# CasualGANPapers/Make-A-Scene

Hardware: AMD Instinct MI355X
Metric: VQ-IMG 256x256 images/sec/node (recon+VQ fwd+bwd) (higher is better)
Workload: dtype bf16; 1 GPU; VQ-IMG 256x256, codebook 8192x256, conf/img_config.yaml model block (95.2 M params), fwd+bwd of L1+q_loss + Adam step; per_gpu_batch=32, global_batch=32, parallelism=dp1, optimizer=mas_hip.optim.Adam (one launch; = torch.optim.Adam's update)

## Files before the change

### include/mas_hip.h

```cpp
#ifndef MAS_HIP_H
#define MAS_HIP_H

#include <stddef.h>
#include <stdint.h>

#ifdef __cplusplus
extern "C" {
#endif

#define MAS_ABI_VERSION 10

enum { MAS_OK = 0, MAS_EINVAL = -1, MAS_EUNSUPPORTED = -2, MAS_ELAUNCH = -3, MAS_EWORKSPACE = -4 };
enum { MAS_F32 = 0, MAS_BF16 = 1 };
enum { MAS_ACT_NONE = 0,
       MAS_ACT_AFFINE = 1,
       MAS_ACT_AFFINE_SILU = 2  };

typedef struct MasConvDesc {
    int32_t N, H, W, Cin;
    int32_t Ho, Wo, Cout;
    int32_t ks;
    int32_t stride;
    int32_t pad_top, pad_left;
    int32_t in_dtype;
    int32_t out_dtype;
    int32_t act;
    int32_t upsample;
    int32_t w_layout;
    int32_t wgrad_cus;
} MasConvDesc;

int         mas_abi_version(void);
const char* mas_last_error(void);
const char* mas_last_kernel(void);

size_t mas_packed_weight_elems(int Cout, int Cin, int ks);
int    mas_pack_conv_weight(const float* w_oihw, void* packed, int Cout, int Cin, int ks,
                            int transpose, int dtype, void* stream);
enum { MAS_WLAYOUT_K64 = 0, MAS_WLAYOUT_K32 = 1, MAS_WLAYOUT_UP2 = 2 };
size_t mas_packed_weight_elems_up2(int Cout, int Cin);
int    mas_conv_weight_layout(const MasConvDesc* d);
int    mas_pack_conv_weight_layout(const float* w_oihw, void* packed, int Cout, int Cin, int ks,
                                   int transpose, int dtype, int layout, void* stream);

typedef struct MasPackItem {
    const float* w_oihw; void* packed;
    int Cout, Cin, ks, transpose, dtype, layout, first_block, n_blocks;
} MasPackItem;
int    mas_pack_batch_blocks(int Cout, int Cin, int ks, int transpose, int dtype, int layout);
int    mas_pack_conv_weight_batch(const MasPackItem* items_device, int n_items, int total_blocks, void* stream);

typedef struct MasPackTileItem {
    const float* w_oihw; void* img[4];
    int transpose[4], layout[4];
    int n_img, Cout, Cin, ks, first_block, pad_;
} MasPackTileItem;
int    mas_pack_tile_blocks(int Cout, int Cin, int ks);
int    mas_pack_conv_weight_tiles(const MasPackTileItem* items_device, int n_items, int total_blocks, int max_ks, void* stream);

typedef struct MasAdamItem {
    float* p; const float* g; float* m; float* v;
    long long n;
    int first_block, pad_;
} MasAdamItem;
int    mas_adam_blocks(long long numel);
int    mas_adam_multi(const MasAdamItem* items_device, int n_items, int total_blocks, float lr, float beta1, float beta2, float eps,
                      float weight_decay, double bias_correction1, double bias_correction2, void* stream);

int    mas_grad_sqnorm_multi(const MasAdamItem* items_device, int n_items, int total_blocks, double* partials, void* stream);
int    mas_grad_clip_coef(const double* partials, int n_partials, const double* extra, int n_extra, float max_norm, float* out, void* stream);
int    mas_adam_multi_ex(const MasAdamItem* items_device, int n_items, int total_blocks, float lr, float beta1, float beta2, float eps,
                         float weight_decay, double bias_correction1, double bias_correction2, const float* grad_scale_device,
                         int decoupled_wd, void* stream);
int    mas_grad_scale_multi(const MasAdamItem* items_device, int n_items, int total_blocks, const float* scale_device, void* stream);

int    mas_adam_multi_ema(const MasAdamItem* items_device, float* const* ema_device, int n_items, int total_blocks, float lr, float beta1,
                          float beta2, float eps, float weight_decay, double bias_correction1, double bias_correction2,
                          const float* grad_scale_device, int decoupled_wd, float ema_decay, const float* grad_norm_device, void* stream);
int    mas_swap_multi(const MasAdamItem* items_device, float* const* other_device, int n_items, int total_blocks, void* stream);

int    mas_adam_multi_dev(const MasAdamItem* items_device, float* const* ema_device, const float* const* step_device, int n_items,
                          int total_blocks, const float* lr_device, double beta1, double beta2, float eps, float weight_decay,
                          const float* grad_scale_device, int decoupled_wd, double ema_decay, const float* ema_count_device,
                          const float* grad_norm_device, float* scalars_device, void* stream);
int    mas_adam_advance_dev(float* counters, int n, void* stream);

size_t mas_gn_stats_workspace(int N, int C);
int    mas_gn_stats(const void* x, int dtype, int N, int HW, int C, int G, float eps,
// ... 267 lines not shown
int mas_obj_head_grid_dev(int level, int max_cells, int n_canvas, int H, int W);
int mas_obj_canvas_fwd_dev(const MasFaceImage* img, const MasFaceImage* rec, const int32_t* table_dev, int max_cells, int n_images,
                           int n_canvas, int H, int W, const float* shift, const float* scale, void* canvas, int dtype, void* stream);
int mas_obj_canvas_bwd_dev(const void* dcanvas, int dtype, const int32_t* table_dev, int max_cells, int n_images, int n_canvas, int H, int W,
                           const float* scale, const MasFaceImage* drec, void* stream);
int mas_obj_relu_fwd_dev(void* y, const int32_t* table_dev, int max_cells, int n_images, int n_canvas, int H, int W, int level, int N, int C,
                         int dtype, void* stream);
int mas_obj_pool_fwd_dev(const void* x, void* y, const int32_t* table_dev, int max_cells, int n_images, int n_canvas, int H, int W, int level,
                         int N, int C, int dtype, void* stream);
int mas_obj_pool_bwd_dev(const void* a, const void* seed, const void* dz, void* dy, const int32_t* table_dev, int max_cells, int n_images,
                         int n_canvas, int H, int W, int level, int N, int C, int dtype, void* stream);
int mas_obj_head_fwd_dev(const void* feat, const float* w, const int32_t* table_dev, int max_cells, int n_images, int n_canvas, int H, int W,
                         int level, int dtype, float* partial, void* stream);
int mas_obj_finalize_dev(const float* partial, const int32_t* table_dev, int max_cells, int n_images, int n_canvas, int H, int W, float* out,
                         void* stream);
int mas_obj_head_bwd_dev(const void* feat, const float* w, const int32_t* table_dev, int max_cells, int n_images, int n_canvas, int H, int W,
                         int level, int dtype, const float* dout, void* seed, void* stream);

int mas_lpips_pack_fwd(const MasFaceImage* real, const MasFaceImage* fake, const float* shift, const float* scale, void* canvas, int dtype,
                       void* stream);
int mas_lpips_pack_bwd(const void* dcanvas, int dtype, const float* scale, const MasFaceImage* dfake, void* stream);
int mas_lpips_relu_fwd(void* y, long long n, int dtype, void* stream);
int mas_lpips_pool_fwd(const void* x, void* y, int N, int H, int W, int C, int dtype, void* stream);
int mas_lpips_pool_bwd(const void* a, const void* seed, const void* dz, void* dy, int N, int H, int W, int C, int dtype, void* stream);
int mas_lpips_head_blocks(int H, int W, int C);
int mas_lpips_head_fwd(const void* feat, const float* w, int B, int H, int W, int C, int dtype, float* partial, void* stream);
int mas_lpips_finalize(const float* partial, int B, int n_levels, const int32_t* hw, const int32_t* blocks, float* out, void* stream);
int mas_lpips_head_bwd(const void* feat, const float* w, int B, int H, int W, int C, int dtype, const float* dout, void* seed, void* stream);

#define MAS_RESERVOIR_PER_IMAGE 10
#define MAS_RESERVOIR_MAX_CANDIDATES 2048
int mas_reservoir_collect(const float* z, float* buf, int32_t* state, int32_t* plan, long long seed, int R, int B, int HW, int D,
                          void* stream);

size_t mas_kmeans_workspace(int M, int K);
int mas_kmeans_init(const float* points, int M, int K, int D, long long seed, int draw, float* centroids, int32_t* init_idx, void* stream);
int mas_kmeans_fit(const float* points, float* centroids, int M, int K, int D, int max_iter, float tol, int64_t* assign, int32_t* info,
                   double* shift, void* workspace, size_t ws_bytes, void* stream);

enum { MAS_GAN_RUN = 8 };
int mas_gan_l1_blocks(int N, int C, int H, int W);
int mas_gan_l1_fwd(const void* img, int img_dtype, int img_layout, const void* rec, int rec_dtype, int rec_layout, int N, int C, int H,
                   int W, double* partials, int n_partials, void* stream);
int mas_gan_l1_finalize(const double* partials, int n_partials, long long numel, const float* perceptual, int B, float perceptual_weight,
                        float* out, void* stream);
int mas_gan_l1_bwd(const void* img, int img_dtype, int img_layout, const void* rec, int rec_dtype, int rec_layout, int N, int C, int H,
                   int W, const float* grad, void* drec, float* dperceptual, int B, float perceptual_weight, void* stream);
int mas_gan_logits_fwd(const float* fake, long long n_fake, const float* real, long long n_real, const long long* global_step,
                       long long disc_start, float disc_factor, float* out, void* stream);
int mas_gan_logits_bwd(const float* fake, long long n_fake, const float* real, long long n_real, const float* grad_gen, const float* grad_d,
                       const float* gate, float* dfake, float* dreal, void* stream);
int mas_gan_combine_fwd(const float* nll, const float* g_loss, const float* codebook, long long n_codebook, const float* face,
                        const float* object, const float* nll_grads, const float* g_grads, long long n_grads, long long* global_step,
                        long long disc_start, float disc_factor, float disc_weight, float codebook_weight, int advance, float* out,
                        void* stream);
int mas_gan_combine_bwd(const float* grad, const float* out, float codebook_weight, long long n_codebook, float* grads, void* stream);

#ifdef __cplusplus
}
#endif
#endif
```

### make-a-scene_amd/csrc/misc.hip

```cpp
#include "mas_common.h"
#include <stdarg.h>

static thread_local char g_err[512] = "";

void mas_set_error(const char* fmt, ...) {
    va_list ap;
    va_start(ap, fmt);
    vsnprintf(g_err, sizeof(g_err), fmt, ap);
    va_end(ap);
}

int mas_num_cus() {
    static std::atomic<int> cus[64];
    int dev = 0;
    if (hipGetDevice(&dev) != hipSuccess) return 256;
    int c = cus[dev & 63].load(std::memory_order_relaxed);
    if (c == 0) {
        int n = 0;
        c = (hipDeviceGetAttribute(&n, hipDeviceAttributeMultiprocessorCount, dev) == hipSuccess && n > 0) ? n : 256;
        cus[dev & 63].store(c, std::memory_order_relaxed);
    }
    return c;
}

// ... 122 lines not shown
    const int b = blockIdx.x;
    while (lo < hi) {
        const int mid = (lo + hi + 1) >> 1;
        if (items[mid].first_block <= b) lo = mid; else hi = mid - 1;
    }
    const MasPackItem it = items[lo];
    const long long first = (long long)(b - it.first_block) * NT + threadIdx.x, stride = (long long)it.n_blocks * NT;
    const int rows = it.transpose ? it.Cin : it.Cout, cols = it.transpose ? it.Cout : it.Cin;
    const int rows_pad = (rows + 127) / 128 * 128;
    auto cdiv = [](int a, int d) { return (a + d - 1) / d; };
    if (it.layout == MAS_WLAYOUT_UP2)
        pack_weight_up2_body(it.w_oihw, (bf16_t*)it.packed, it.Cout, it.Cin, it.transpose, rows_pad, cdiv(cols, 32), first, stride);
    else if (it.layout == MAS_WLAYOUT_K32)
        pack_weight_k32_body(it.w_oihw, (bf16_t*)it.packed, it.Cout, it.Cin, it.ks, it.transpose, rows_pad, cdiv(cols, 32), first, stride);
    else if (it.dtype == MAS_BF16)
        pack_weight_body<bf16_t>(it.w_oihw, (bf16_t*)it.packed, it.Cout, it.Cin, it.ks, it.transpose, rows_pad, cdiv(cols, 64), first, stride);
    else
        pack_weight_body<float>(it.w_oihw, (float*)it.packed, it.Cout, it.Cin, it.ks, it.transpose, rows_pad, cdiv(cols, 32), first, stride);
}

__device__ __forceinline__ unsigned pk2(const bf16_t* l, int a, int b) {
    return (unsigned)reinterpret_cast<const unsigned short*>(l)[a] | ((unsigned)reinterpret_cast<const unsigned short*>(l)[b] << 16);
}
__global__ __launch_bounds__(NT) void pack_weight_tiles_kernel(const MasPackTileItem* __restrict__ items, int n_items) {
    extern __shared__ __attribute__((aligned(16))) unsigned char tsm[];
    bf16_t* L = reinterpret_cast<bf16_t*>(tsm);
    int lo = 0, hi = n_items - 1;
    const int b = blockIdx.x, tid = threadIdx.x;
    while (lo < hi) {
        const int mid = (lo + hi + 1) >> 1;
        if (items[mid].first_block <= b) lo = mid; else hi = mid - 1;
    }
    const MasPackTileItem it = items[lo];
    const int Cout = it.Cout, Cin = it.Cin, kk = it.ks * it.ks;
    const int tiles_i = (Cin + 127) / 128 * 2;
    const int tb = b - it.first_block, o0 = (tb / tiles_i) * 64, i0 = (tb % tiles_i) * 64;
    const int run = 64 * kk;
    const bool full = i0 + 64 <= Cin && ((size_t)Cin * kk) % 4 == 0 && (reinterpret_cast<uintptr_t>(it.w_oihw) & 15) == 0;
    if (full) {
        const int v4 = run / 4;
        for (int u = tid; u < 64 * v4; u += NT) {
            const int ol = u / v4, q = u - ol * v4;
            f32x4 v = {0.0f, 0.0f, 0.0f, 0.0f};
            if (o0 + ol < Cout) v = *reinterpret_cast<const f32x4*>(it.w_oihw + ((size_t)(o0 + ol) * Cin + i0) * kk + 4 * q);
            const bf16x4 o = {(bf16_t)v[0], (bf16_t)v[1], (bf16_t)v[2], (bf16_t)v[3]};
            *reinterpret_cast<bf16x4*>(L + (size_t)ol * run + 4 * q) = o;
        }
    } else {
        const int valid = i0 < Cin ? (Cin - i0 < 64 ? Cin - i0 : 64) * kk : 0;
        for (int u = tid; u < 64 * run; u += NT) {
            const int ol = u / run, f = u - ol * run;
            float v = 0.0f;
            if (o0 + ol < Cout && f < valid) v = it.w_oihw[((size_t)(o0 + ol) * Cin + i0) * kk + f];
            L[u] = (bf16_t)v;
        }
    }
    __syncthreads();
    for (int im = 0; im < it.n_img; ++im) {
        const int tr = it.transpose[im], k32 = it.layout[im] == MAS_WLAYOUT_K32;
        const int rows = tr ? Cin : Cout, cols = tr ? Cout : Cin;
        const int r0 = tr ? i0 : o0, c0 = tr ? o0 : i0;
        const int rows_pad = (rows + 127) / 128 * 128;
        if (r0 >= rows_pad) continue;
        unsigned char* out = reinterpret_cast<unsigned char*>(it.img[im]);
        if (!k32) {
            const int ch = c0 / 64;
            if (ch >= (cols + 63) / 64) continue;
            for (int u = tid; u < kk * 512; u += NT) {
                const int t = u >> 9, row_l = (u >> 3) & 63, sp = u & 7;
                const int row = r0 + row_l, ls = sp ^ ((row >> 1) & 7);
                const int ts = tr ? kk - 1 - t : t;
                u32x4 o;
#pragma unroll
                for (int e = 0; e < 4; ++e) {
                    const int ca = ls * 8 + 2 * e, cb = ca + 1;
                    const int ia = tr ? (ca * 64 + row_l) * kk + ts : (row_l * 64 + ca) * kk + ts;
                    const int ib = tr ? (cb * 64 + row_l) * kk + ts : (row_l * 64 + cb) * kk + ts;
                    o[e] = pk2(L, ia, ib);
                }
                *reinterpret_cast<u32x4*>(out + ((size_t)(ch * kk + t) * rows_pad + row) * 128 + sp * 16) = o;
            }
        } else {
            const int half = (r0 >> 6) & 1, base = r0 & ~127;
            for (int h = 0; h < 2; ++h) {
                const int ch = c0 / 32 + h;
                if (ch >= (cols + 31) / 32) continue;
                for (int u = tid; u < kk * 256; u += NT) {
                    const int t = u >> 8, i_ = (u >> 6) & 3, l16 = (u >> 2) & 15, sp = u & 3;
                    const int row = base + 32 * i_ + l16 + 16 * half;
                    const int row_l = 4 * l16 + i_;
                    const int ls = sp ^ ((row >> 2) & 3);
                    const int ts = tr ? kk - 1 - t : t;
                    u32x4 o;
#pragma unroll
                    for (int e = 0; e < 4; ++e) {
                        const int ca = h * 32 + ls * 8 + 2 * e, cb = ca + 1;
                        const int ia = tr ? (ca * 64 + row_l) * kk + ts : (row_l * 64 + ca) * kk + ts;
                        const int ib = tr ? (cb * 64 + row_l) * kk + ts : (row_l * 64 + cb) * kk + ts;
                        o[e] = pk2(L, ia, ib);
                    }
                    *reinterpret_cast<u32x4*>(out + ((size_t)(ch * kk + t) * rows_pad + row) * 64 + sp * 16) = o;
                }
            }
        }
    }
}

template <typename T>
__global__ __launch_bounds__(NT) void upsample2x_kernel(const T* __restrict__ x, T* __restrict__ y, int N, int H, int W, int C) {
    constexpr int EPU = 16 / (int)sizeof(T);
    const int upp = C / EPU;
    const long long total = (long long)N * 2 * H * 2 * W * upp;
    for (long long i = (long long)blockIdx.x * NT + threadIdx.x; i < total; i += (long long)gridDim.x * NT) {
// ... 380 lines not shown
```

### make-a-scene_amd/csrc/reservoir.hip

```cpp
#include "mas_common.h"
#include "mas_philox.h"

#define RSV_THREADS 256

MAS_HD uint32_t rsv_half_bits(uint32_t N);
#include "mas_bijection.h"

__device__ __forceinline__ int rsv_scan(int mine, int* s_scan) {
    __syncthreads();
    s_scan[threadIdx.x] = mine;
    __syncthreads();
    if (threadIdx.x == 0) {
        int run = 0;
        for (int i = 0; i < RSV_THREADS; ++i) { const int v = s_scan[i]; s_scan[i] = run; run += v; }
    }
    __syncthreads();
    return s_scan[threadIdx.x];
}

__global__ __launch_bounds__(RSV_THREADS) void reservoir_plan_kernel(int* __restrict__ state, int* __restrict__ plan, uint32_t k0, uint32_t k1,
                                                                     int R, int B, int HW) {
    __shared__ int s_drop[MAS_RESERVOIR_MAX_CANDIDATES];
    __shared__ int s_old[MAS_RESERVOIR_MAX_CANDIDATES];
    __shared__ int s_list[MAS_RESERVOIR_MAX_CANDIDATES];
// ... 40 lines not shown
    const int i = blockIdx.x * (RSV_THREADS / 64) + (threadIdx.x >> 6), lane = threadIdx.x & 63;
    if (i >= n) return;
    const int dst = plan[2 * i], src = plan[2 * i + 1];
    if (dst < 0 || dst >= R || src < 0 || src >= rows) return;
    const f32x4* from = reinterpret_cast<const f32x4*>(z + (size_t)src * D);
    f32x4* to = reinterpret_cast<f32x4*>(buf + (size_t)dst * D);
    for (int q = lane; q < D / 4; q += 64) to[q] = from[q];
}

extern "C" int mas_reservoir_collect(const float* z, float* buf, int32_t* state, int32_t* plan, long long seed, int R, int B, int HW, int D,
                                     void* stream) {
    MAS_ENTER();
    if (HW < MAS_RESERVOIR_PER_IMAGE) MAS_FAIL(MAS_EINVAL, "reservoir_collect: %d latent positions, fewer than the %d drawn per image", HW,
                                               MAS_RESERVOIR_PER_IMAGE);
    if (B <= 0 || R <= 0 || (long long)MAS_RESERVOIR_PER_IMAGE * B > R)
        MAS_FAIL(MAS_EINVAL, "reservoir_collect: %d candidates per call (10 * B, B=%d) exceed the reservoir's %d rows", 10 * B, B, R);
    if (D <= 0 || D % 4) MAS_FAIL(MAS_EINVAL, "reservoir_collect: D=%d is not a positive multiple of 4 (16-byte row copies)", D);
    if (MAS_RESERVOIR_PER_IMAGE * B > MAS_RESERVOIR_MAX_CANDIDATES)
        MAS_FAIL(MAS_EUNSUPPORTED, "reservoir_collect: B=%d gives more than %d candidates per call", B, MAS_RESERVOIR_MAX_CANDIDATES);
    if ((long long)R + MAS_RESERVOIR_PER_IMAGE * B > (1ll << 30) || (long long)B * HW > (1ll << 30))
        MAS_FAIL(MAS_EUNSUPPORTED, "reservoir_collect: R=%d, B*HW=%lld beyond 2^30 rows", R, (long long)B * HW);
    if (!z || !buf || !state || !plan) MAS_FAIL(MAS_EINVAL, "reservoir_collect: null argument");
    if (((uintptr_t)z | (uintptr_t)buf) & 15) MAS_FAIL(MAS_EINVAL, "reservoir_collect: z and buf must be 16-byte aligned");
    const int n = MAS_RESERVOIR_PER_IMAGE * B;
    hipStream_t s = reinterpret_cast<hipStream_t>(stream);
    hipLaunchKernelGGL(reservoir_plan_kernel, dim3(1), dim3(RSV_THREADS), 0, s, state, plan, (uint32_t)((unsigned long long)seed & 0xffffffffu),
                       (uint32_t)((unsigned long long)seed >> 32), R, B, HW);
    MAS_CHECK_LAUNCH("reservoir_plan");
    hipLaunchKernelGGL(reservoir_copy_kernel, dim3(mas_cdiv(n, RSV_THREADS / 64)), dim3(RSV_THREADS), 0, s, z, buf, plan, n, R,
                       (long long)B * HW, D);
    MAS_CHECK_LAUNCH("reservoir_copy");
    return MAS_OK;
}
```

### make-a-scene_amd/mas_hip/__init__.py

```python
from __future__ import annotations

import ctypes as C
import os
import threading

os.environ.setdefault("GPU_MAX_HW_QUEUES", "8")

import torch

from . import _header

_HERE = os.path.dirname(os.path.abspath(__file__))
LIB_PATH = os.environ.get("MAS_HIP_LIB") or os.path.join(_HERE, "libmas_hip.so")


class ConvDesc(C.Structure):
    _fields_ = [(n, C.c_int32) for n in (
        "N", "H", "W", "Cin", "Ho", "Wo", "Cout", "ks", "stride", "pad_top", "pad_left",
        "in_dtype", "out_dtype", "act", "upsample", "w_layout", "wgrad_cus")]


class PackItem(C.Structure):
    _fields_ = [("w_oihw", C.c_void_p), ("packed", C.c_void_p)] + [(n, C.c_int32) for n in (
        "Cout", "Cin", "ks", "transpose", "dtype", "layout", "first_block", "n_blocks")]


class PackTileItem(C.Structure):
    _fields_ = [("w_oihw", C.c_void_p), ("img", C.c_void_p * 4), ("transpose", C.c_int32 * 4), ("layout", C.c_int32 * 4)] + \
               [(n, C.c_int32) for n in ("n_img", "Cout", "Cin", "ks", "first_block", "pad_")]


class AdamItem(C.Structure):
    _fields_ = [("p", C.c_void_p), ("g", C.c_void_p), ("m", C.c_void_p), ("v", C.c_void_p), ("n", C.c_longlong), ("first_block", C.c_int32),
                ("pad_", C.c_int32)]


class FaceRow(C.Structure):
    _fields_ = [(n, C.c_int32) for n in ("src", "b", "top", "left", "h", "w", "rh", "rw", "ct", "cl")]


class FaceImage(C.Structure):
    _fields_ = [("data", C.c_void_p)] + [(n, C.c_int32) for n in ("dtype", "N", "C", "H", "W", "pad_")] + \
               [(n, C.c_int64) for n in ("sn", "sc", "sh", "sw")]


class FaceBnItem(C.Structure):
    _fields_ = [(n, C.c_void_p) for n in ("weight", "bias", "mean", "var")] + [("C", C.c_int32), ("off", C.c_int32), ("eps", C.c_float),
                                                                                ("pad_", C.c_int32)]


class FaceFeats(C.Structure):
    _fields_ = [("p", C.c_void_p * 5), ("chw", C.c_int32 * 5), ("half", C.c_int32), ("dtype", C.c_int32), ("alpha", C.c_float * 5)]


class ObjCell(C.Structure):
    _fields_ = [(n, C.c_int32) for n in ("n", "oy", "ox", "h", "w", "b", "top", "left")]


class ObjPlan(C.Structure):
    _fields_ = [("cells", C.c_void_p), ("img_cell0", C.c_void_p), ("tiles", C.c_void_p), ("blk0", C.c_void_p)] + \
               [(n, C.c_int32) for n in ("n_cells", "n_images", "n_canvas", "H", "W", "pad_")]

# ... 63 lines not shown
```

### make-a-scene_amd/mas_hip/ops.py

```python
from __future__ import annotations

import contextlib
import ctypes as C
import os
import weakref
from typing import Optional

import torch

from . import ACT_AFFINE, ACT_AFFINE_SILU, ACT_NONE, ATTN_DECODE_MAX_SPLITS, BF16, F32, IMG_SSIM_WINDOW, SEG_NCHW, SEG_NHWC, SEG_U8, WLAYOUT_K64, \
    WLAYOUT_UP2, ConvDesc, PackItem, PackTileItem, _DT, _ptr, _require_cuda, _stream, check, lib
from .seglabels import SegLabels

_state = {"compute_dtype": torch.bfloat16 if os.environ.get("MAS_COMPUTE_DTYPE", "bf16") == "bf16" else torch.float32}


def compute_dtype() -> torch.dtype:
    return _state["compute_dtype"]


def set_compute_dtype(dt: torch.dtype) -> None:
    if dt not in _DT:
        raise ValueError("compute dtype must be torch.bfloat16 or torch.float32")
    _state["compute_dtype"] = dt
# ... 36 lines not shown
            _param_generation[k] = _param_generation.get(k, 0) + 1


try:
    from torch.optim.optimizer import register_optimizer_step_post_hook as _register_post_hook
    _register_post_hook(_note_optimizer_step)
except ImportError:
    _orig_opt_step = torch.optim.Optimizer.step

    def _step_and_note(self, *a, **k):
        out = _orig_opt_step(self, *a, **k)
        _note_optimizer_step(self)
        return out

    torch.optim.Optimizer.step = _step_and_note


def _param_stamp(p: torch.Tensor):
    return (p._version, p.data_ptr(), _param_generation.get(id(p), 0))


_CACHE_CHECK = os.environ.get("MAS_WEIGHT_CACHE_CHECK", "0") == "1"


def _checksum(w: torch.Tensor) -> float:
    return float(w.detach().double().sum())


class _PackCache:

    def __init__(self):
        self.store = {}
        self.derived = {}
        self.sums = {}
        self._tables = {}

    def clear(self):
        self.store.clear()
        self.derived.clear()
        self._tables.clear()

    def drop(self, w: torch.Tensor):
        k = id(w)
        for key in [key for key in self.store if key[0] == k]:
            self.store.pop(key, None)
        for key in [key for key in self.derived if k in key[0]]:
            self.derived.pop(key, None)

    def get_derived(self, w: torch.Tensor, sources, transpose: bool, dtype: torch.dtype, layout: int) -> torch.Tensor:
        key = (tuple(id(p) for p in sources), transpose, dtype, layout)
        stamp = tuple(_param_stamp(p) for p in sources)
        hit = self.derived.get(key)
        if hit is not None and hit[1] == stamp and all(r() is p for r, p in zip(hit[0], sources)) and hit[2].device == w.device:
            return hit[2]
        packed = pack_conv_weight(w.detach(), transpose, dtype, layout)
        refs = tuple(weakref.ref(p, lambda _r, k=key: self.derived.pop(k, None)) for p in sources)
        self.derived[key] = (refs, stamp, packed)
        return packed

    def get(self, w: torch.Tensor, transpose: bool, dtype: torch.dtype, layout: int = WLAYOUT_K64, sources=None) -> torch.Tensor:
        if not isinstance(w, torch.nn.Parameter):
            if sources is not None:
                return self.get_derived(w, sources, transpose, dtype, layout)
            return pack_conv_weight(w.detach(), transpose, dtype, layout)
        key = (id(w), transpose, dtype, layout)
        hit = self.store.get(key)
        if hit is not None and hit[0]() is w and hit[1] == _param_stamp(w):
            if _CACHE_CHECK and self.sums.get(key) != _checksum(w):
                raise RuntimeError("packed-weight cache: parameter of shape %s changed without a version bump / optimizer step (a write "
                                   "through .data?) -- call mas_hip.ops.invalidate_weight_cache() after such writes" % (tuple(w.shape),))
            return hit[2]
        if hit is None or hit[0]() is not w or hit[2].device != w.device:
            n = _packed_elems(w.shape[0], w.shape[1], w.shape[2], layout)
            self.store[key] = [weakref.ref(w, lambda _r, k=key: self.store.pop(k, None)), None, torch.empty(n, dtype=dtype, device=w.device)]
        self.refresh_stale(w.device)
        return self.store[key][2]

    def tensors(self):
        return [e[2] for e in self.store.values()] + [e[2] for e in self.derived.values()] + [t[1] for t in self._tables.values()]

    def forget_stamps(self):
        for e in self.store.values():
            e[1] = None
        self.derived.clear()

    def refresh_stale(self, device):
        groups, items, first, fresh, keep = {}, [], 0, [], []
        for key, ent in list(self.store.items()):
            wid, transpose, dtype, layout = key
            w = ent[0]()
            if w is None or w.device != device or ent[1] == _param_stamp(w):
                continue
            cout, cin, ks, _ = w.shape
            wf = w.detach()
            if wf.dtype != torch.float32 or not wf.is_contiguous():
                wf = wf.contiguous().float()
                keep.append(wf)
            ent[1] = None
            fresh.append((ent, _param_stamp(w)))
            if _CACHE_CHECK:
                self.sums[key] = _checksum(w)
            g = groups.get(wid)
            if dtype == torch.bfloat16 and ks <= 4 and layout != WLAYOUT_UP2 and (g is None or len(g[2]) < 4):
                if g is None:
                    g = groups[wid] = (wf, (cout, cin, ks), [])
                g[2].append((ent[2].data_ptr(), int(transpose), int(layout)))
                continue
            nb = lib().mas_pack_batch_blocks(cout, cin, ks, int(transpose), _DT[dtype], int(layout))
            if nb <= 0:
                raise RuntimeError(f"pack_conv_weight: unsupported weight shape {tuple(w.shape)}")
            items.append(PackItem(wf.data_ptr(), ent[2].data_ptr(), cout, cin, ks, int(transpose), _DT[dtype], int(layout), first, nb))
            first += nb
        if groups:
            titems, tfirst, max_ks = [], 0, 1
            for wf, (cout, cin, ks), imgs in groups.values():
                it = PackTileItem()
                it.w_oihw, it.n_img, it.Cout, it.Cin, it.ks, it.first_block = wf.data_ptr(), len(imgs), cout, cin, ks, tfirst
                for k, (ptr, tr, lay) in enumerate(imgs):
                    it.img[k], it.transpose[k], it.layout[k] = ptr, tr, lay
                titems.append(it)
                tfirst += lib().mas_pack_tile_blocks(cout, cin, ks)
                max_ks = max(max_ks, ks)
            table = self._upload("tiles", device, (PackTileItem * len(titems))(*titems))
            check(lib().mas_pack_conv_weight_tiles(_ptr(table), len(titems), tfirst, max_ks, _stream()), "pack_conv_weight_tiles")
        if items:
            table = self._upload("batch", device, (PackItem * len(items))(*items))
            check(lib().mas_pack_conv_weight_batch(_ptr(table), len(items), first, _stream()), "pack_conv_weight_batch")
        for ent, stamp in fresh:
            ent[1] = stamp

    def _upload(self, which, device, arr):
        raw = bytes(memoryview(arr))
        sig = (device.index, raw)
        hit = self._tables.get(which)
        if hit is None or hit[0] != sig:
            if torch.cuda.is_current_stream_capturing():
                raise RuntimeError("packed-weight cache: a graph capture would upload a new item table (a copy from pageable memory, which a "
                                   "capture cannot hold): refresh the same set of stale images once before capturing, as GraphedTrainStep does")
            hit = self._tables[which] = (sig, torch.frombuffer(bytearray(raw), dtype=torch.uint8).to(device))
        return hit[1]


_pack_cache = _PackCache()


def drop_weight_cache_of(*params) -> None:
    for p in params:
# ... 617 lines not shown

def norm_act_conv(x, weight, bias, gn_w=None, gn_b=None, residual=None, *, stride=1, padding=(1, 1, 1, 1), act=ACT_NONE,
                  upsample=False, groups=32, eps=1e-6, in_dtype=None, out_dtype=None):
    cd = in_dtype or compute_dtype()
    cfg = dict(stride=stride, pad_top=padding[0], pad_bottom=padding[1], pad_left=padding[2], pad_right=padding[3], act=act,
               upsample=bool(upsample), groups=groups, eps=eps, in_dtype=cd, out_dtype=out_dtype or cd, grad=torch.is_grad_enabled())
    if cfg["in_dtype"] == torch.float32 and cfg["out_dtype"] != torch.float32:
        raise RuntimeError("conv: fp32 input requires fp32 output")
    epu = 8 if cd == torch.bfloat16 else 4
    cout, cin = weight.shape[0], weight.shape[1]
    if isinstance(x, SegLabels):
        if act != ACT_NONE:
            raise RuntimeError("conv: SegLabels feed a plain convolution only (no GroupNorm in front)")
        if x.shape[1] != cin:
            raise ValueError(f"conv: SegLabels of {x.shape[1]} channels ({x.layout}), weight expects {cin}")
        padc = (epu - cin % epu) % epu
        x = seg_expand(x, dtype=cd, channels_last=True, pad_to=cin + padc)
        if padc:
            weight = torch.nn.functional.pad(weight, (0, 0, 0, 0, 0, padc))
    elif act == ACT_NONE and cin % epu:
        padc = epu - cin % epu
        x = torch.nn.functional.pad(nhwc(x, cd), (0, 0, 0, 0, 0, padc))
        weight = torch.nn.functional.pad(weight, (0, 0, 0, 0, 0, padc))
    if cout % epu and residual is None:
        padc = epu - cout % epu
        weight = torch.nn.functional.pad(weight, (0, 0, 0, 0, 0, 0, 0, padc))
        if bias is not None:
            bias = torch.nn.functional.pad(bias, (0, padc))
        return _NormActConv.apply(x, weight, bias, gn_w, gn_b, residual, cfg)[:, :cout]
    xpart, xrows = _take_stats(x) if act != ACT_NONE else (None, 0)
    return _attach_stats(_NormActConv.apply(x, weight, bias, gn_w, gn_b, residual, cfg, xpart, xrows))


class _ResBlock(torch.autograd.Function):

    @staticmethod
    def forward(ctx, x, n1w, n1b, c1w, c1b, n2w, n2b, c2w, c2b, sw, sb, groups, eps, cd, xpart=None, xrows=0, grad=True):
        _require_cuda(x, "resblock")
        x = nhwc(x, cd)
        n, c, h, w = x.shape
        co = c1w.shape[0]
        f32 = lambda t: t.detach().float() if t is not None else None
        ng = ctx.needs_input_grad
        mat = _MATERIALIZE and _gn_act_ok(c, x.dtype) and _gn_act_ok(co, x.dtype)

        def norm(inp, gw, gb, part, rows):
            if mat and part is None and gn_small_ok(inp, groups):
                return gn_stats_act(inp, f32(gw), f32(gb), groups, eps, ACT_AFFINE_SILU)
            return gn_stats(inp, f32(gw), f32(gb), groups, eps, part, rows) + (None,)

        def conv(inp, ss_, a_, wgt, bia, resid, need_w, ci):
            if mat:
                if a_ is None:
                    a_ = gn_act(inp, ss_, ACT_AFFINE_SILU)
                return conv_fwd_raw(a_, None, ConvWeight(wgt, False), f32(bia), resid, n, h, w, ci, h, w, co, 3, 1, 1, 1, ACT_NONE, False, cd,
                                    want_stats=True) + (a_ if grad and need_w and _save_act["on"] else None,)
            return conv_fwd_raw(inp, ss_, ConvWeight(wgt, False), f32(bia), resid, n, h, w, ci, h, w, co, 3, 1, 1, 1, ACT_AFFINE_SILU, False,
                                cd, want_stats=True) + (None,)

        mr1, ss1, act1 = norm(x, n1w, n1b, xpart, xrows)
        hh, hpart, hrows, a1 = conv(x, ss1, act1, c1w, c1b, None, ng[3] or ng[4], c)
        skip = x if sw is None else conv_fwd_raw(x, None, ConvWeight(sw, False), f32(sb), None, n, h, w, c, h, w, co, 1, 1, 0, 0, ACT_NONE, False, cd)
        mr2, ss2, act2 = norm(hh, n2w, n2b, hpart, hrows)
        y, ypart, yrows, a2 = conv(hh, ss2, act2, c2w, c2b, skip, ng[7] or ng[8], co)
        _stats_state["stash"] = (ypart, yrows) if ypart is not None else None
        ctx.groups, ctx.cd, ctx.has_sc = groups, cd, sw is not None
# ... 125 lines not shown


def reservoir_plan_elems(batch_size: int) -> int:
    return 2 * RESERVOIR_PER_IMAGE * int(batch_size)


def reservoir_collect(z, buf, state, seed, plan=None):
    if z.dim() == 4:
        b, d, hw = z.shape[0], z.shape[1], z.shape[2] * z.shape[3]
        flat = z.permute(0, 2, 3, 1)
    elif z.dim() == 3:
        b, hw, d = z.shape
        flat = z
    else:
        raise ValueError(f"reservoir_collect: z must be [B, D, H, W] or [B, HW, D], got {tuple(z.shape)}")
    if buf.dim() != 2 or buf.shape[1] != d:
        raise ValueError(f"reservoir_collect: buf {tuple(buf.shape)} against latent rows of {d} elements")
    r = buf.shape[0]
    if hw < RESERVOIR_PER_IMAGE or RESERVOIR_PER_IMAGE * b > r or d % 4 or b < 1:
        raise ValueError(f"reservoir_collect: needs HW >= {RESERVOIR_PER_IMAGE}, 10 * B <= R and D % 4 == 0; got B={b}, HW={hw}, D={d}, R={r}")
    _require_cuda(z, "reservoir_collect")
    if not (flat.is_contiguous() and z.dtype == torch.float32 and buf.dtype == torch.float32 and buf.is_contiguous() and buf.device == z.device):
        raise RuntimeError("reservoir_collect: z must be fp32 in NHWC memory and buf a contiguous fp32 tensor on the same device")
    if not (state.dtype == torch.int32 and state.numel() >= 2 and state.is_contiguous() and state.device == z.device):
        raise RuntimeError("reservoir_collect: state must be a contiguous int32 tensor {rows held, calls} on z's device")
    if plan is None:
        plan = torch.empty(reservoir_plan_elems(b), dtype=torch.int32, device=z.device)
    elif not (plan.dtype == torch.int32 and plan.numel() >= reservoir_plan_elems(b) and plan.is_contiguous() and plan.device == z.device):
        raise RuntimeError(f"reservoir_collect: plan must be a contiguous int32 tensor of at least {reservoir_plan_elems(b)} elements on z's device")
    seed = int(seed) & 0xFFFFFFFFFFFFFFFF
    check(lib().mas_reservoir_collect(_ptr(z), _ptr(buf), _ptr(state), _ptr(plan), seed - (1 << 64) if seed >= 1 << 63 else seed, r, b, hw, d,
                                      _stream()), "reservoir_collect")
    return plan


def _signed64(seed) -> int:
    seed = int(seed) & 0xFFFFFFFFFFFFFFFF
    return seed - (1 << 64) if seed >= 1 << 63 else seed


def _kmeans_points(points, n_clusters, who: str):
    if points.dim() != 2:
        raise ValueError(f"{who}: points must be [M, D], got {tuple(points.shape)}")
    m, d = points.shape
    k = int(n_clusters)
    if d < 1 or d > _VQ_DIMS[-1]:
        raise ValueError(f"{who}: D={d} outside the kernel envelope: widths up to {_VQ_DIMS[-1]} (instantiated for {_VQ_DIMS}, narrower "
                         f"ones zero-padded)")
    if k < 1 or k > m:
        raise ValueError(f"{who}: needs 1 <= n_clusters <= M distinct rows, got n_clusters={k}, M={m}")
    if m > 1 << 30:
        raise ValueError(f"{who}: M={m} beyond 2^30 rows")
    _require_cuda(points, who)
    pts = points.detach().float()
    if d not in _VQ_DIMS:
        pts = torch.nn.functional.pad(pts, (0, next(v for v in _VQ_DIMS if v >= d) - d))
    pts = pts.contiguous()
    if pts.data_ptr() % 16:
        raise ValueError(f"{who}: points must be 16-byte aligned (the kernels read rows with 16-byte loads); the storage offset is "
                         f"{points.storage_offset()} elements")
    return pts, d


def kmeans_init(points, n_clusters, seed, draw=0):
    pts, d = _kmeans_points(points, n_clusters, "kmeans_init")
    k = int(n_clusters)
# ... 1265 lines not shown
```

### make-a-scene_amd/models/modules.py

```python
from __future__ import annotations

import contextlib
import os

import torch
import torch.nn as nn
import torch.nn.functional as F
import torch.distributed as dist

from mas_hip import ACT_AFFINE, ACT_AFFINE_SILU, ACT_NONE
from mas_hip import ops

_MAS_SYNCBN = int(os.environ.get("MAS_SYNCBN", "2"))
_EXCHANGE_AT_WORLD_1 = os.environ.get("MAS_SYNCBN_EXCHANGE_AT_WORLD_1", "0") == "1"
_RESERVOIR_ASYNC = os.environ.get("MAS_RESERVOIR_ASYNC", "1") == "1"
_DEVICE_RESERVOIR = os.environ.get("MAS_DEVICE_RESERVOIR", "0") == "1"


def nonlinearity(x):
    return x * torch.sigmoid(x)


class _GroupNorm(nn.GroupNorm):
    """GroupNorm(32, C, eps=1e-6).  Inside Encoder/Decoder/ResnetBlock/AttnBlock its parameters are
# ... 114 lines not shown

    def forward(self, x):
        if self.training and self.dropout.p > 0:
            h = self.conv1.fused(x, self.norm1, ACT_AFFINE_SILU)
            a = ops.dropout(ops.group_norm_act(h, self.norm2, ACT_AFFINE_SILU, dtype=h.dtype), self.dropout.p, True)
            if self.in_channels != self.out_channels:
                x = self.conv_shortcut(x) if self.use_conv_shortcut else self.nin_shortcut(x)
            return self.conv2(a, residual=x)
        plain = self.conv1.in_dtype is None and self.conv2.out_dtype is None and self.conv1.bias is not None and self.conv2.bias is not None
        if plain and self.in_channels == self.out_channels:
            return ops.resblock(x, self.norm1, self.conv1, self.norm2, self.conv2)
        if plain and not self.use_conv_shortcut and self.nin_shortcut.bias is not None and self.nin_shortcut.in_dtype is None \
                and self.nin_shortcut.out_dtype is None and self.in_channels % 64 == 0 and self.out_channels % 128 == 0:
            return ops.resblock(x, self.norm1, self.conv1, self.norm2, self.conv2, self.nin_shortcut)
        h = self.conv1.fused(x, self.norm1, ACT_AFFINE_SILU)
        if self.in_channels != self.out_channels:
            x = self.conv_shortcut(x) if self.use_conv_shortcut else self.nin_shortcut(x)
        return self.conv2.fused(h, self.norm2, ACT_AFFINE_SILU, residual=x)


class AttnBlock(nn.Module):

    def __init__(self, in_channels):
        super().__init__()
        self.in_channels = in_channels
        self.norm = Normalize(in_channels)
        self.q = Conv2d(in_channels, in_channels, kernel_size=1, stride=1, padding=0)
        self.k = Conv2d(in_channels, in_channels, kernel_size=1, stride=1, padding=0)
        self.v = Conv2d(in_channels, in_channels, kernel_size=1, stride=1, padding=0)
        self.proj_out = Conv2d(in_channels, in_channels, kernel_size=1, stride=1, padding=0)

    def forward(self, x):
        c = self.in_channels
        w_qkv = torch.cat([self.q.weight, self.k.weight, self.v.weight], dim=0)
        w_qkv._mas_sources = (self.q.weight, self.k.weight, self.v.weight)
        b_qkv = torch.cat([self.q.bias, self.k.bias, self.v.bias], dim=0)
        qkv = ops.norm_act_conv(x, w_qkv, b_qkv, self.norm.weight, self.norm.bias, None, stride=1, padding=(0, 0, 0, 0),
                                act=ACT_AFFINE, groups=self.norm.num_groups, eps=self.norm.eps)
        h_ = ops.spatial_attention(qkv, c)
        return self.proj_out(h_, residual=x)


class Swish(nn.Module):
    def forward(self, x):
        return x * torch.sigmoid(x)


def _run_layers(layers, x):
    layers = list(layers)
    i = 0
    while i < len(layers):
        m = layers[i]
        if isinstance(m, _GroupNorm) and i + 2 < len(layers) + 0 and isinstance(layers[i + 1], Swish) and isinstance(layers[i + 2], Conv2d):
            x = layers[i + 2].fused(x, m, ACT_AFFINE_SILU)
            i += 3
        else:
            x = m(x)
            i += 1
    return x


class Encoder(nn.Module):

    def __init__(self, in_channels=3, channels=[128, 128, 128, 256, 512, 512], attn_resolutions=[32], resolution=512, dropout=0.0,
                 num_res_blocks=2, z_channels=256, **kwargs):
        super(Encoder, self).__init__()
# ... 123 lines not shown

    @contextlib.contextmanager
    def ticked_by_caller(self):
        old, self._ticked_outside = self._ticked_outside, True
        try:
            yield
        finally:
            self._ticked_outside = old

    @contextlib.contextmanager
    def dry_forward(self):
        c = self._dev["c"]
        try:
            yield
        finally:
            self._dev["c"], self.reservoir = c, self._dev["buf"][:c]

    def rows_per_call(self):
        return self._dev.get("last_n", 0) if self.training and self.phase() >= 1 else 0

    @staticmethod
    def _randperm(n, device, keep=None):
        p = torch.randperm(n)
        if keep is not None:
            p = p[:keep]
        if device.type != "cuda" or not _RESERVOIR_ASYNC:
            return p.to(device)
        pinned = torch.empty(p.numel(), dtype=p.dtype, pin_memory=True)
        pinned.copy_(p)
        return pinned.to(device, non_blocking=True)

    def _collect(self, z_flat, batch_size):
        z_new = z_flat.detach().reshape(batch_size, -1, self.codebook_dim)
        z_new = z_new[:, self._randperm(z_new.size(1), z_new.device)][:, :10].reshape(-1, self.codebook_dim)
        self.reservoir = z_new if self.reservoir is None else torch.cat([self.reservoir, z_new], dim=0)
        keep = self._randperm(self.reservoir.size(0), self.reservoir.device, self.reservoir_size)
        self.reservoir = self.reservoir[keep].detach()

    def _reinit_from_reservoir(self):
        from .kmeans import kmeans_fit
        distributed = dist.is_available() and dist.is_initialized()
        world_size = dist.get_world_size() if distributed else 1
        print("Updating codebook from reservoir.")
        if world_size > 1:
            gathered = [torch.zeros_like(self.reservoir) for _ in range(world_size)]
            dist.all_gather(gathered, self.reservoir.clone())
            pool = torch.cat(gathered, dim=0)
        else:
            pool = self.reservoir
        if self._dev is not None and self._dev["device_kmeans"]:
            cent = kmeans_fit(pool, self.codebook_size, on_device=True, seed=self._dev["seed"], draw=self.q_counter)
        elif self._dev is not None:
            det, warn = torch.are_deterministic_algorithms_enabled(), torch.is_deterministic_algorithms_warn_only_enabled()
            torch.use_deterministic_algorithms(True, warn_only=True)
            try:
                cent = kmeans_fit(pool, self.codebook_size)
            finally:
                torch.use_deterministic_algorithms(det, warn_only=warn)
        else:
            cent = kmeans_fit(pool, self.codebook_size)
        cent = cent.detach().contiguous()
        if world_size > 1:
            dist.broadcast(cent, 0)
        if self._dev is not None:
            self.embedding.weight.data.copy_(cent)
        else:
# ... 38 lines not shown
```

Baseline: 618.3 images/s.

## Pack QKV weights directly into stacked image and fuse reservoir gather

Adds a stacked packed-weight cache for the attention q/k/v 1x1 convs. The pack kernel writes each source Parameter straight into its slice of one forward and one transposed packed image, and copies the biases into a shared fp32 vector. This avoids the per-step torch.cat of weights and biases and lets a new autograd function split the gradients back per Parameter. It also replaces the reservoir's gather/cat/gather chain with one device kernel that picks rows from the old buffer or the new latents, removing several intermediate tensors and launches. The cost is more code paths and cache bookkeeping, plus bounds checks inside the gather kernel.

```diff
diff --git a/include/mas_hip.h b/include/mas_hip.h
--- a/include/mas_hip.h
+++ b/include/mas_hip.h
@@ -53,7 +53,7 @@
 typedef struct MasPackTileItem {
     const float* w_oihw; void* img[4];
     int transpose[4], layout[4];
-    int n_img, Cout, Cin, ks, first_block, pad_;
+    int n_img, Cout, Cin, ks, first_block, stack_rows;
 } MasPackTileItem;
 int    mas_pack_tile_blocks(int Cout, int Cin, int ks);
 int    mas_pack_conv_weight_tiles(const MasPackTileItem* items_device, int n_items, int total_blocks, int max_ks, void* stream);
@@ -387,6 +387,8 @@
 #define MAS_RESERVOIR_MAX_CANDIDATES 2048
 int mas_reservoir_collect(const float* z, float* buf, int32_t* state, int32_t* plan, long long seed, int R, int B, int HW, int D,
                           void* stream);
+int mas_reservoir_gather(const float* z, const float* old, const int64_t* perm, const int64_t* keep, float* out, int n_keep, int n_old,
+                         int B, int HW, int D, void* stream);
 
 size_t mas_kmeans_workspace(int M, int K);
 int mas_kmeans_init(const float* points, int M, int K, int D, long long seed, int draw, float* centroids, int32_t* init_idx, void* stream);
diff --git a/make-a-scene_amd/csrc/misc.hip b/make-a-scene_amd/csrc/misc.hip
--- a/make-a-scene_amd/csrc/misc.hip
+++ b/make-a-scene_amd/csrc/misc.hip
@@ -178,6 +178,11 @@
         if (items[mid].first_block <= b) lo = mid; else hi = mid - 1;
     }
     const MasPackTileItem it = items[lo];
+    if (it.n_img == 0) {
+        float* dst = reinterpret_cast<float*>(it.img[0]);
+        for (int u = tid; u < it.Cout; u += NT) dst[u] = it.w_oihw[u];
+        return;
+    }
     const int Cout = it.Cout, Cin = it.Cin, kk = it.ks * it.ks;
     const int tiles_i = (Cin + 127) / 128 * 2;
     const int tb = b - it.first_block, o0 = (tb / tiles_i) * 64, i0 = (tb % tiles_i) * 64;
@@ -212,6 +217,7 @@
         if (!k32) {
             const int ch = c0 / 64;
             if (ch >= (cols + 63) / 64) continue;
+            const int row_stride = !tr && it.stack_rows > 0 ? it.stack_rows : rows_pad;
             for (int u = tid; u < kk * 512; u += NT) {
                 const int t = u >> 9, row_l = (u >> 3) & 63, sp = u & 7;
                 const int row = r0 + row_l, ls = sp ^ ((row >> 1) & 7);
@@ -224,7 +230,7 @@
                     const int ib = tr ? (cb * 64 + row_l) * kk + ts : (row_l * 64 + cb) * kk + ts;
                     o[e] = pk2(L, ia, ib);
                 }
-                *reinterpret_cast<u32x4*>(out + ((size_t)(ch * kk + t) * rows_pad + row) * 128 + sp * 16) = o;
+                *reinterpret_cast<u32x4*>(out + ((size_t)(ch * kk + t) * row_stride + row) * 128 + sp * 16) = o;
             }
         } else {
             const int half = (r0 >> 6) & 1, base = r0 & ~127;
diff --git a/make-a-scene_amd/csrc/reservoir.hip b/make-a-scene_amd/csrc/reservoir.hip
--- a/make-a-scene_amd/csrc/reservoir.hip
+++ b/make-a-scene_amd/csrc/reservoir.hip
@@ -96,3 +96,42 @@
     MAS_CHECK_LAUNCH("reservoir_copy");
     return MAS_OK;
 }
+
+__global__ __launch_bounds__(RSV_THREADS) void reservoir_gather_kernel(const float* __restrict__ z, const float* __restrict__ old,
+                                                                       const long long* __restrict__ perm, const long long* __restrict__ keep,
+                                                                       float* __restrict__ out, int n_keep, int n_old, int B, int HW, int D) {
+    const int i = blockIdx.x * (RSV_THREADS / 64) + (threadIdx.x >> 6), lane = threadIdx.x & 63;
+    if (i >= n_keep) return;
+    const long long k = keep[i];
+    if (k < 0 || k >= (long long)n_old + (long long)MAS_RESERVOIR_PER_IMAGE * B) return;
+    const float* src;
+    if (k < n_old) src = old + (size_t)k * D;
+    else {
+        const int c = (int)(k - n_old);
+        const long long p = perm[c % MAS_RESERVOIR_PER_IMAGE];
+        if (p < 0 || p >= HW) return;
+        src = z + ((size_t)(c / MAS_RESERVOIR_PER_IMAGE) * HW + (size_t)p) * D;
+    }
+    const f32x4* from = reinterpret_cast<const f32x4*>(src);
+    f32x4* to = reinterpret_cast<f32x4*>(out + (size_t)i * D);
+    for (int q = lane; q < D / 4; q += 64) to[q] = from[q];
+}
+
+extern "C" int mas_reservoir_gather(const float* z, const float* old, const int64_t* perm, const int64_t* keep, float* out, int n_keep, int n_old,
+                                    int B, int HW, int D, void* stream) {
+    MAS_ENTER();
+    if (HW < MAS_RESERVOIR_PER_IMAGE) MAS_FAIL(MAS_EINVAL, "reservoir_gather: %d latent positions, fewer than the %d drawn per image", HW,
+                                               MAS_RESERVOIR_PER_IMAGE);
+    if (B <= 0 || n_old < 0 || n_keep <= 0 || (long long)n_keep > (long long)n_old + (long long)MAS_RESERVOIR_PER_IMAGE * B)
+        MAS_FAIL(MAS_EINVAL, "reservoir_gather: keeps %d rows of %d held + 10 * %d new", n_keep, n_old, B);
+    if (D <= 0 || D % 4) MAS_FAIL(MAS_EINVAL, "reservoir_gather: D=%d is not a positive multiple of 4 (16-byte row copies)", D);
+    if ((long long)n_old + (long long)MAS_RESERVOIR_PER_IMAGE * B > (1ll << 30) || (long long)B * HW > (1ll << 30))
+        MAS_FAIL(MAS_EUNSUPPORTED, "reservoir_gather: %d rows held, B*HW=%lld beyond 2^30 rows", n_old, (long long)B * HW);
+    if (!z || !perm || !keep || !out || (n_old > 0 && !old)) MAS_FAIL(MAS_EINVAL, "reservoir_gather: null argument");
+    if (((uintptr_t)z | (uintptr_t)old | (uintptr_t)out) & 15) MAS_FAIL(MAS_EINVAL, "reservoir_gather: z, old and out must be 16-byte aligned");
+    if (((uintptr_t)perm | (uintptr_t)keep) & 7) MAS_FAIL(MAS_EINVAL, "reservoir_gather: perm and keep must be 8-byte aligned int64");
+    hipLaunchKernelGGL(reservoir_gather_kernel, dim3(mas_cdiv(n_keep, RSV_THREADS / 64)), dim3(RSV_THREADS), 0, reinterpret_cast<hipStream_t>(stream),
+                       z, old, reinterpret_cast<const long long*>(perm), reinterpret_cast<const long long*>(keep), out, n_keep, n_old, B, HW, D);
+    MAS_CHECK_LAUNCH("reservoir_gather");
+    return MAS_OK;
+}
diff --git a/make-a-scene_amd/mas_hip/__init__.py b/make-a-scene_amd/mas_hip/__init__.py
--- a/make-a-scene_amd/mas_hip/__init__.py
+++ b/make-a-scene_amd/mas_hip/__init__.py
@@ -27,7 +27,7 @@
 
 class PackTileItem(C.Structure):
     _fields_ = [("w_oihw", C.c_void_p), ("img", C.c_void_p * 4), ("transpose", C.c_int32 * 4), ("layout", C.c_int32 * 4)] + \
-               [(n, C.c_int32) for n in ("n_img", "Cout", "Cin", "ks", "first_block", "pad_")]
+               [(n, C.c_int32) for n in ("n_img", "Cout", "Cin", "ks", "first_block", "stack_rows")]
 
 
 class AdamItem(C.Structure):
diff --git a/make-a-scene_amd/mas_hip/ops.py b/make-a-scene_amd/mas_hip/ops.py
--- a/make-a-scene_amd/mas_hip/ops.py
+++ b/make-a-scene_amd/mas_hip/ops.py
@@ -92,12 +92,14 @@
     def __init__(self):
         self.store = {}
         self.derived = {}
+        self.stacks = {}
         self.sums = {}
         self._tables = {}
 
     def clear(self):
         self.store.clear()
         self.derived.clear()
+        self.stacks.clear()
         self._tables.clear()
 
     def drop(self, w: torch.Tensor):
@@ -106,6 +108,8 @@
             self.store.pop(key, None)
         for key in [key for key in self.derived if k in key[0]]:
             self.derived.pop(key, None)
+        for key in [key for key, ent in self.stacks.items() if any(r() is w for r in ent[0])]:
+            self.stacks.pop(key, None)
 
     def get_derived(self, w: torch.Tensor, sources, transpose: bool, dtype: torch.dtype, layout: int) -> torch.Tensor:
         key = (tuple(id(p) for p in sources), transpose, dtype, layout)
@@ -117,6 +121,27 @@
         refs = tuple(weakref.ref(p, lambda _r, k=key: self.derived.pop(k, None)) for p in sources)
         self.derived[key] = (refs, stamp, packed)
         return packed
+
+    def get_stacked(self, weights, biases, dtype: torch.dtype):
+        params = tuple(weights) + tuple(biases)
+        w0 = weights[0]
+        c = w0.shape[0]
+        if dtype != torch.bfloat16 or len(weights) != 3 or len(biases) != 3 or c % 128 or not all(isinstance(p, torch.nn.Parameter) for p in params) \
+                or any(tuple(w.shape) != (c, c, 1, 1) for w in weights) or any(tuple(b.shape) != (c,) for b in biases) \
+                or any(p.device != w0.device for p in params):
+            raise RuntimeError("packed-weight cache: a stacked image takes three [C, C, 1, 1] Parameters, C % 128 == 0, and their [C] biases, in bf16")
+        key = (tuple(id(w) for w in weights), dtype)
+        hit = self.stacks.get(key)
+        if hit is not None and all(r() is p for r, p in zip(hit[0], params)) and hit[2].device == w0.device:
+            if hit[1] == tuple(_param_stamp(p) for p in params):
+                return hit[2], hit[3], hit[4]
+        else:
+            refs = tuple(weakref.ref(p, lambda _r, k=key: self.stacks.pop(k, None)) for p in params)
+            n = _packed_elems(3 * c, c, 1, WLAYOUT_K64)
+            hit = self.stacks[key] = [refs, None, torch.empty(n, dtype=dtype, device=w0.device), torch.empty(n, dtype=dtype, device=w0.device),
+                                      torch.empty(3 * c, dtype=torch.float32, device=w0.device)]
+        self.refresh_stale(w0.device)
+        return hit[2], hit[3], hit[4]
 
     def get(self, w: torch.Tensor, transpose: bool, dtype: torch.dtype, layout: int = WLAYOUT_K64, sources=None) -> torch.Tensor:
         if not isinstance(w, torch.nn.Parameter):
@@ -137,10 +162,10 @@
         return self.store[key][2]
 
     def tensors(self):
-        return [e[2] for e in self.store.values()] + [e[2] for e in self.derived.values()] + [t[1] for t in self._tables.values()]
+        return [e[2] for e in self.store.values()] + [e[2] for e in self.derived.values()] + [t for e in self.stacks.values() for t in e[2:]] + [t[1] for t in self._tables.values()]
 
     def forget_stamps(self):
-        for e in self.store.values():
+        for e in list(self.store.values()) + list(self.stacks.values()):
             e[1] = None
         self.derived.clear()
 
@@ -171,8 +196,43 @@
                 raise RuntimeError(f"pack_conv_weight: unsupported weight shape {tuple(w.shape)}")
             items.append(PackItem(wf.data_ptr(), ent[2].data_ptr(), cout, cin, ks, int(transpose), _DT[dtype], int(layout), first, nb))
             first += nb
-        if groups:
+        stacked = []
+        for ent in list(self.stacks.values()):
+            params = [r() for r in ent[0]]
+            if any(p is None for p in params) or params[0].device != device:
+                continue
+            stamp = tuple(_param_stamp(p) for p in params)
+            if ent[1] == stamp:
+                continue
+            ent[1] = None
+            fresh.append((ent, stamp))
+            c = params[0].shape[0]
+            for i, p in enumerate(params):
+                pf = p.detach()
+                if pf.dtype != torch.float32 or not pf.is_contiguous():
+                    pf = pf.contiguous().float()
+                    keep.append(pf)
+                if i < 3:
+                    esz = ent[2].element_size()
+                    stacked.append((pf, 3 * c, [(ent[2].data_ptr() + i * c * 64 * esz, 0, int(WLAYOUT_K64)),
+                                                (ent[3].data_ptr() + i * (c // 64) * c * 64 * esz, 1, int(WLAYOUT_K64))]))
+                else:
+                    stacked.append((pf, 0, ent[4].data_ptr() + (i - 3) * c * 4))
+        if groups or stacked:
             titems, tfirst, max_ks = [], 0, 1
+            for pf, stack_rows, imgs in stacked:
+                it = PackTileItem()
+                if stack_rows:
+                    c = pf.shape[0]
+                    it.w_oihw, it.n_img, it.Cout, it.Cin, it.ks, it.first_block, it.stack_rows = pf.data_ptr(), len(imgs), c, c, 1, tfirst, stack_rows
+                    for k, (ptr, tr, lay) in enumerate(imgs):
+                        it.img[k], it.transpose[k], it.layout[k] = ptr, tr, lay
+                    tfirst += lib().mas_pack_tile_blocks(c, c, 1)
+                else:
+                    it.w_oihw, it.n_img, it.Cout, it.first_block = pf.data_ptr(), 0, pf.shape[0], tfirst
+                    it.img[0] = imgs
+                    tfirst += 1
+                titems.append(it)
             for wf, (cout, cin, ks), imgs in groups.values():
                 it = PackTileItem()
                 it.w_oihw, it.n_img, it.Cout, it.Cin, it.ks, it.first_block = wf.data_ptr(), len(imgs), cout, cin, ks, tfirst
@@ -856,6 +916,92 @@
     return _attach_stats(_NormActConv.apply(x, weight, bias, gn_w, gn_b, residual, cfg, xpart, xrows))
 
 
+class _NormQKV(torch.autograd.Function):
+
+    @staticmethod
+    def forward(ctx, x, qw, kw, vw, qb, kb, vb, gn_w, gn_b, groups, eps, grad, xpart=None, xrows=0):
+        _require_cuda(x, "qkv")
+        cd = torch.bfloat16
+        x = nhwc(x, cd)
+        n, c, h, w = x.shape
+        act = ACT_AFFINE
+        wp, _, b32 = _pack_cache.get_stacked((qw, kw, vw), (qb, kb, vb), cd)
+        mat = _MATERIALIZE and _CONV1X1 and _gn_act_ok(c, cd)
+        a = None
+        if mat and xpart is None and gn_small_ok(x, groups):
+            mr, ss, a = gn_stats_act(x, gn_w.detach().float(), gn_b.detach().float(), groups, eps, act)
+        else:
+            mr, ss = gn_stats(x, gn_w.detach().float(), gn_b.detach().float(), groups, eps, xpart, xrows)
+        need_wgrad = grad and any(ctx.needs_input_grad[1:7])
+        if mat:
+            if a is None:
+                a = gn_act(x, ss, act)
+            y, ypart, yrows = conv_fwd_raw(a, None, wp, b32, None, n, h, w, c, h, w, 3 * c, 1, 1, 0, 0, ACT_NONE, False, cd, want_stats=True)
+            if not need_wgrad or not _save_act["on"]:
+                a = None
+        else:
+            y, ypart, yrows = conv_fwd_raw(x, ss, wp, b32, None, n, h, w, c, h, w, 3 * c, 1, 1, 0, 0, act, False, cd, want_stats=True)
+        _stats_state["stash"] = (ypart, yrows) if ypart is not None else None
+        ctx.groups, ctx.dims = groups, (n, h, w, c)
+        ctx.save_for_backward(x, qw, kw, vw, qb, kb, vb, gn_w, mr, ss, a)
+        return y
+
+    @staticmethod
+    def backward(ctx, dy):
+        x, qw, kw, vw, qb, kb, vb, gn_w, mr, ss, a = ctx.saved_tensors
+        n, h, w, c = ctx.dims
+        cd, act = torch.bfloat16, ACT_AFFINE
+        dy = nhwc(dy, cd)
+        need_x, need_w, need_b = ctx.needs_input_grad[0], any(ctx.needs_input_grad[1:4]), any(ctx.needs_input_grad[4:7])
+        need_gn = ctx.needs_input_grad[7] or ctx.needs_input_grad[8]
+        dx = dw = db = dgw = dgb = None
+
+        def wgrad(*outs):
+            if a is not None:
+                return conv_wgrad_raw(a, None, dy, n, h, w, c, h, w, 3 * c, 1, 1, 0, 0, ACT_NONE, False, need_b, *outs)
+            return conv_wgrad_raw(x, ss, dy, n, h, w, c, h, w, 3 * c, 1, 1, 0, 0, act, False, need_b, *outs)
+
+        defer = (need_w or need_b) and (need_x or need_gn) and x.numel() >= _WGRAD_STREAM_MIN_ELEMS and _side_stream_on()
+        if (need_w or need_b) and not defer:
+            dw, db = wgrad()
+        if need_x or need_gn:
+            _, wt, _ = _pack_cache.get_stacked((qw, kw, vw), (qb, kb, vb), cd)
+            da = conv_fwd_raw(dy, None, wt, None, None, n, h, w, 3 * c, h, w, c, 1, 1, 0, 0, ACT_NONE, False, cd)
+            with _side_section(defer) as on_side:
+                if defer:
+                    outs = (torch.empty((3 * c, c, 1, 1), dtype=torch.float32, device=x.device),
+                            torch.empty(3 * c, dtype=torch.float32, device=x.device) if need_b else None)
+                    dw, db = on_side(lambda: wgrad(*outs))
+                dx, dgw, dgb = gn_bwd(x, da, None, ctx.groups, act, gn_w.detach().float(), mr, ss)
+                dgw, dgb = dgw.to(gn_w.dtype), dgb.to(gn_w.dtype)
+        dws = [None] * 3 if dw is None or not need_w else [dw.view(3, c, c, 1, 1)[i].to(p.dtype) for i, p in enumerate((qw, kw, vw))]
+        dbs = [None] * 3 if db is None else [db.view(3, c)[i].to(p.dtype) for i, p in enumerate((qb, kb, vb))]
+        for i in range(3):
+            if not ctx.needs_input_grad[1 + i]:
+                dws[i] = None
+            if not ctx.needs_input_grad[4 + i]:
+                dbs[i] = None
+        return (dx, *dws, *dbs, dgw, dgb, None, None, None, None, None)
+
+
+_qkv_state = {"sources": True}
+
+
+def set_qkv_sources(on: bool) -> bool:
+    old, _qkv_state["sources"] = _qkv_state["sources"], bool(on)
+    return old
+
+
+def qkv_sources_ok(x: torch.Tensor, c: int) -> bool:
+    return _qkv_state["sources"] and x.is_cuda and compute_dtype() == torch.bfloat16 and c % 128 == 0
+
+
+def norm_qkv(x, q, k, v, norm):
+    xpart, xrows = _take_stats(x)
+    return _attach_stats(_NormQKV.apply(x, q.weight, k.weight, v.weight, q.bias, k.bias, v.bias, norm.weight, norm.bias, norm.num_groups,
+                                        norm.eps, torch.is_grad_enabled(), xpart, xrows))
+
+
 class _ResBlock(torch.autograd.Function):
 
     @staticmethod
@@ -1047,6 +1193,27 @@
     check(lib().mas_reservoir_collect(_ptr(z), _ptr(buf), _ptr(state), _ptr(plan), seed - (1 << 64) if seed >= 1 << 63 else seed, r, b, hw, d,
                                       _stream()), "reservoir_collect")
     return plan
+
+
+def reservoir_gather(z, old, perm, keep):
+    _require_cuda(z, "reservoir_gather")
+    if z.dim() != 3:
+        raise ValueError(f"reservoir_gather: z must be [B, HW, D], got {tuple(z.shape)}")
+    b, hw, d = z.shape
+    n_old = 0 if old is None else old.shape[0]
+    n_keep = keep.numel()
+    if hw < RESERVOIR_PER_IMAGE or d % 4 or b < 1 or not 0 < n_keep <= n_old + RESERVOIR_PER_IMAGE * b or perm.numel() < RESERVOIR_PER_IMAGE:
+        raise ValueError(f"reservoir_gather: needs HW >= {RESERVOIR_PER_IMAGE}, D % 4 == 0, 10 positions and 0 < len(keep) <= n_old + 10 * B; "
+                         f"got B={b}, HW={hw}, D={d}, n_old={n_old}, {perm.numel()} positions, {n_keep} kept")
+    if not (z.is_contiguous() and z.dtype == torch.float32 and (old is None or (old.dim() == 2 and old.shape[1] == d and old.is_contiguous()
+                                                                                and old.dtype == torch.float32 and old.device == z.device))):
+        raise RuntimeError("reservoir_gather: z and the old reservoir must be contiguous fp32 tensors of D-element rows on one device")
+    if not all(t.dtype == torch.int64 and t.dim() == 1 and t.is_contiguous() and t.device == z.device for t in (perm, keep)):
+        raise RuntimeError("reservoir_gather: perm and keep must be contiguous int64 vectors on z's device")
+    out = torch.empty((n_keep, d), dtype=torch.float32, device=z.device)
+    check(lib().mas_reservoir_gather(_ptr(z), _ptr(old) if n_old else None, _ptr(perm), _ptr(keep), _ptr(out), n_keep, n_old, b, hw, d, _stream()),
+          "reservoir_gather")
+    return out
 
 
 def _signed64(seed) -> int:
diff --git a/make-a-scene_amd/models/modules.py b/make-a-scene_amd/models/modules.py
--- a/make-a-scene_amd/models/modules.py
+++ b/make-a-scene_amd/models/modules.py
@@ -170,6 +170,8 @@
 
     def forward(self, x):
         c = self.in_channels
+        if ops.qkv_sources_ok(x, c):
+            return self.proj_out(ops.spatial_attention(ops.norm_qkv(x, self.q, self.k, self.v, self.norm), c), residual=x)
         w_qkv = torch.cat([self.q.weight, self.k.weight, self.v.weight], dim=0)
         w_qkv._mas_sources = (self.q.weight, self.k.weight, self.v.weight)
         b_qkv = torch.cat([self.q.bias, self.k.bias, self.v.bias], dim=0)
@@ -359,6 +361,13 @@
 
     def _collect(self, z_flat, batch_size):
         z_new = z_flat.detach().reshape(batch_size, -1, self.codebook_dim)
+        if z_new.is_cuda and z_new.dtype == torch.float32 and z_new.is_contiguous() and self.codebook_dim % 4 == 0 and z_new.size(1) >= 10 \
+                and (self.reservoir is None or (self.reservoir.is_contiguous() and self.reservoir.dtype == torch.float32)):
+            perm = self._randperm(z_new.size(1), z_new.device, 10)
+            n_old = 0 if self.reservoir is None else self.reservoir.size(0)
+            keep = self._randperm(n_old + 10 * batch_size, z_new.device, self.reservoir_size)
+            self.reservoir = ops.reservoir_gather(z_new, self.reservoir, perm, keep)
+            return
         z_new = z_new[:, self._randperm(z_new.size(1), z_new.device)][:, :10].reshape(-1, self.codebook_dim)
         self.reservoir = z_new if self.reservoir is None else torch.cat([self.reservoir, z_new], dim=0)
         keep = self._randperm(self.reservoir.size(0), self.reservoir.device, self.reservoir_size)
```

New measurement: 620.4 images/s, median of 6. About the same (+0.4%).
